# mirage/decompress

Measured on AMD Instinct MI355X. Metric: MiB/s inflate over N zlib streams (uncompressed bytes / wall second), higher is better.
Workload: dtype u8

## Files before the change

decompress_amd/csrc/inflate_wave.hip:

```cpp
#include <stdlib.h>
#include <string.h>
#include "inflate_util.hpp"

namespace md {
namespace wv {

constexpr uint32_t S = 264;
constexpr uint32_t SMIN = 48;
constexpr uint32_t KMAX = 64;
#ifndef MD_EMIT_SPLIT
#define MD_EMIT_SPLIT 1
#endif
#if defined(MD_DEBUG_KNOWN_BOUNDS)
#undef MD_EMIT_SPLIT
#define MD_EMIT_SPLIT 0
#endif
#ifndef MD_SPLIT_B
#define MD_SPLIT_B 4
#endif
#ifndef MD_RUNIN_NUM
#define MD_RUNIN_NUM 3
#define MD_RUNIN_DEN 2
#endif
constexpr uint32_t RUNIN_NUM = MD_RUNIN_NUM, RUNIN_DEN = MD_RUNIN_DEN;
constexpr uint32_t PASSES = 5;
constexpr uint32_t PASS_BITS = 1600, PASSES_MAX = 16;
constexpr uint32_t RMAX = 768;
constexpr uint32_t STAGE = 5568;
constexpr uint32_t WIN_WORDS = 544;

constexpr uint32_t kLitSize = 852, kDistSize = 592;
constexpr uint32_t kLitRootMax = 512;
constexpr uint32_t kLitSubB = 0;
constexpr uint32_t kDistB = kLitSize - kLitRootMax;
constexpr uint32_t kLitB = kDistB + kDistSize;
constexpr uint32_t kStopEobI = kLitB + kLitRootMax;
constexpr uint32_t kStopBadI = kStopEobI + 2;
constexpr uint32_t kLutWords = kStopBadI + 2;
constexpr uint32_t kTbMask = 0xffe00000u;
constexpr uint32_t kLoopy = 0x100u;
static_assert(kDistB % 2 == 0 && kLitB % 2 == 0 && kStopEobI % 2 == 0 && kLutWords == 1448, "even table bases");
constexpr uint32_t kStEob = 100, kStTrunc = 101;
constexpr uint32_t kCountMatch = 1u << 20;
constexpr uint32_t kNearBit = 0x8000u;

struct Mail {
  uint32_t emitted;
  uint32_t copied;
  uint32_t kind;
  uint32_t total;
  uint32_t x;
  uint32_t stuck;
  uint32_t a, b;
};
constexpr uint32_t kJobRound = 0, kJobStored = 1, kJobQuit = 2, kJobEmit = 3;
constexpr uint32_t kHxUni = 4 * 64;
struct Smem {
  uint32_t win[WIN_WORDS];
  uint32_t lut[kLutWords];
  uint32_t mrec[RMAX];
  uint16_t mpos[RMAX];
  alignas(16) uint8_t stage[STAGE + 16];
  uint16_t list[RMAX];
  Mail mail;
};
struct HScratch {
  uint8_t lens[384];
  uint16_t work[320];
  uint32_t ctr;
};
static_assert(sizeof(Smem) <= 20480, "8 streams (16 wavefronts) per CU");
constexpr uint32_t kHScratchAt = 1136;
static_assert(kHScratchAt >= 4 + 572 + 8 && kHScratchAt % 16 == 0 && kHScratchAt + sizeof(HScratch) <= WIN_WORDS * 4, "header scratch lives behind the header's bits");
typedef MD_LDS Smem lds_smem;
typedef MD_LDS HScratch lds_hscratch;
__device__ __forceinline__ lds_hscratch *hscratch_of(lds_smem *sm) {
  return reinterpret_cast<lds_hscratch *>(reinterpret_cast<lds_u8 *>(sm->win) + kHScratchAt);
}

#ifdef MD_DEBUG_KNOWN_BOUNDS
constexpr uint32_t KB_ROUNDS = 512;
__device__ uint4 *g_kb_buf;
__device__ int g_kb_mode;
#endif
__device__ __forceinline__ uint32_t mk_entry(uint32_t n, uint32_t xb, uint32_t val8, uint32_t nbits, uint32_t tb) {
  return n | (xb << 5) | (val8 << 9) | (nbits << 17) | (tb << 21);
}
__device__ __forceinline__ uint32_t e_n(uint32_t e) { return e & 31; }
__device__ __forceinline__ uint32_t e_xb(uint32_t e) { return (e >> 5) & 15; }
__device__ __forceinline__ uint32_t e_val(uint32_t e) { return (e >> 9) & 255; }
__device__ __forceinline__ uint32_t e_tb(uint32_t e) { return e >> 21; }
__device__ __forceinline__ bool e_link(uint32_t e) { return e_tb(e) < kLitB && e_tb(e) != kDistB; }
__device__ __forceinline__ uint32_t e_root(uint32_t lroot) { return mk_entry(0, 0, 0, lroot, kLitB); }
__device__ __forceinline__ uint32_t lit_leaf(uint32_t sym, uint32_t codelen, uint32_t lroot, uint32_t droot) {
  if (sym < 256) return mk_entry(codelen, 0, sym, lroot, kLitB);
  if (sym == 256) return mk_entry(codelen, 0, 0, 0, kStopEobI);
  const uint32_t l = (sym - 257) & 31;
  const uint32_t xb = (l >= 8 && l < 28) ? (l - 4) >> 2 : 0;
  const uint32_t base3 = l < 8 ? l : l < 28 ? (4 + (l & 3)) << xb : l == 28 ? 255 : 0;
  return mk_entry(codelen + xb, xb, base3, droot, kDistB);
}
__device__ __forceinline__ uint32_t dist_leaf(uint32_t dv, uint32_t codelen, uint32_t lroot) {
  dv &= 31;
  if (dv >= 30) return mk_entry(codelen, 0, 0, 0, kStopBadI);
  const uint32_t xb = dv >= 4 ? (dv - 2) >> 1 : 0;
  const uint32_t m = dv < 4 ? dv : ((dv & 1) | 2);
  return mk_entry(codelen + xb, xb, m, lroot, kLitB);
}
__device__ __forceinline__ uint32_t dist_value(uint32_t m, uint32_t xb, uint32_t x) { return (m << xb) + 1 + x; }

struct Window {
  uint32_t w[8], wx;
  uint32_t base;
#ifdef MD_DEBUG_KNOWN_BOUNDS
  uint32_t kb_round, kb_sid;
#endif
  __device__ __forceinline__ void fetch(const uint8_t *__restrict__ body, uint32_t nbytes, uint32_t b, uint32_t lane) {
    base = b;
    const uint32_t off = b + lane * 32;
#pragma unroll
    for (int k = 0; k < 8; k++) w[k] = 0;
    if (off + 32 <= nbytes) __builtin_memcpy(w, body + off, 32);
    else if (off < nbytes)
      for (uint32_t k = 0; k < 32 && off + k < nbytes; k++) w[k >> 2] |= (uint32_t)body[off + k] << (8 * (k & 3));
    wx = 0;
    if (lane < WIN_WORDS - 512) {
      const uint32_t ox = b + 2048 + lane * 4;
      if (ox + 4 <= nbytes) __builtin_memcpy(&wx, body + ox, 4);
      else if (ox < nbytes)
        for (uint32_t k = 0; k < 4 && ox + k < nbytes; k++) wx |= (uint32_t)body[ox + k] << (8 * k);
    }
  }
  __device__ __forceinline__ void put(lds_u32 *win, uint32_t lane) const {
    lds_u32 *dst = win + lane * 8;
#pragma unroll
    for (int k = 0; k < 8; k++) dst[k] = w[k];
    if (lane < WIN_WORDS - 512) win[512 + lane] = wx;
  }
  __device__ __forceinline__ void ensure(lds_u32 *win, const uint8_t *__restrict__ body, uint32_t nbytes, uint32_t b, uint32_t lane) {
    if (base != b) fetch(body, nbytes, b, lane);
    put(win, lane);
    base = 0xffffffffu;
  }
};
__device__ __forceinline__ uint32_t peek(const lds_u32 *win, uint32_t p) {
  const lds_u32 *q = reinterpret_cast<const lds_u32 *>(reinterpret_cast<const lds_u8 *>(win) + ((p >> 3) & ~3u));
  return __builtin_amdgcn_alignbit(q[1], q[0], p & 31);
}
__device__ __forceinline__ uint32_t lut_at(const lds_u32 *lut, uint32_t tb, uint32_t idx) {
  return *reinterpret_cast<const lds_u32 *>(reinterpret_cast<const lds_u8 *>(lut) + ((tb + idx) << 2));
}

struct UBits {
  const lds_u32 *win;
  uint64_t buf;
  uint32_t n;
  uint32_t wp;
  __device__ __forceinline__ void init(const lds_u32 *w, uint32_t bp) {
    win = w;
    wp = bp >> 5;
    buf = ((uint64_t)uni(win[wp]) | ((uint64_t)uni(win[wp + 1]) << 32)) >> (bp & 31);
    n = 64 - (bp & 31);
    wp += 2;
  }
  __device__ __forceinline__ uint32_t pos() const { return wp * 32 - n; }
  __device__ __forceinline__ void fill() {
    if (n <= 32) {
      buf |= (uint64_t)uni(win[wp]) << n;
      n += 32;
      wp++;
    }
  }
  __device__ __forceinline__ uint32_t peekb(uint32_t k) const { return (uint32_t)buf & ((1u << k) - 1); }
  __device__ __forceinline__ void drop(uint32_t k) {
    buf >>= k;
    n -= k;
  }
};

struct Canon {
  uint32_t cnt[16];
  uint32_t first[16];
  uint32_t offs[16];
  uint32_t max, min, root, left;
};
__device__ __forceinline__ uint32_t lane_rank(uint64_t m) {
  return __builtin_amdgcn_mbcnt_hi((uint32_t)(m >> 32), __builtin_amdgcn_mbcnt_lo((uint32_t)m, 0));
}
template <int K>
__device__ __forceinline__ void canon_counts(const uint32_t (&len)[K], uint32_t rootpref, Canon &c) {
#pragma unroll
  for (int l = 1; l < 16; l++) {
    uint32_t n = 0;
#pragma unroll
    for (int k = 0; k < K; k++) n += (uint32_t)__builtin_popcountll(__ballot(len[k] == (uint32_t)l));
    c.cnt[l] = n;
  }
  c.cnt[0] = 0;
  c.max = 0;
  c.min = 16;
#pragma unroll
  for (int l = 15; l >= 1; l--) {
    if (c.cnt[l] && c.max == 0) c.max = l;
    if (c.cnt[l]) c.min = l;
  }
  int left = 1;
  bool over = false;
  uint32_t code = 0, off = 0;
  c.first[0] = 0;
  c.offs[0] = 0;
#pragma unroll
  for (int l = 1; l < 16; l++) {
    left = (left << 1) - (int)c.cnt[l];
    over = over || left < 0;
    code = (code + c.cnt[l - 1]) << 1;
    c.first[l] = code;
    c.offs[l] = off;
    off += c.cnt[l];
  }
  c.left = over ? 0xffffffffu : (uint32_t)left;
  uint32_t root = rootpref;
  if (root > c.max) root = c.max;
  if (root < c.min) root = c.min;
  c.root = root;
// ... 319 lines not shown
  uint32_t e = lut_step(lut, e_root(lroot), w);
  if (e_link(e)) {
    p += e_n(e);
    w = peek(win, p);
    e = lut_step(lut, e, w);
  }
  uint32_t n = e_n(e), xb = e_xb(e), ntb = e_tb(e);
  uint32_t pn = p + n;
  if (pn > tot) return MD_UNEXPECTED_END_OF_INPUT;
  if (ntb == kStopEobI) return kStEob | (pn << 8);
  if (ntb != kDistB) {
    if (q >= cap) return MD_UNEXPECTED_END_OF_OUTPUT;
    return kStTrunc;
  }
  const uint32_t mlen = e_val(e) + 3 + __builtin_amdgcn_ubfe(w, n - xb, xb);
  p = pn;
  w = peek(win, p);
  e = lut_step(lut, e, w);
  if (e_tb(e) == kStopBadI && e_n(e) == 0) return MD_INVALID_DISTANCE_CODE;
  if (e_link(e)) {
    p += e_n(e);
    w = peek(win, p);
    e = lut_step(lut, e, w);
  }
  n = e_n(e), xb = e_xb(e);
  pn = p + n;
  if (pn > tot) return MD_UNEXPECTED_END_OF_INPUT;
  if (e_tb(e) == kStopBadI) return MD_INVALID_DISTANCE_CODE;
  const uint32_t d = dist_value(e_val(e), xb, __builtin_amdgcn_ubfe(w, n - xb, xb));
  const uint32_t lim = q < 32768u ? q : 32768u;
  if (d > lim) return MD_INVALID_DISTANCE;
  if (mlen > cap - q) return MD_UNEXPECTED_END_OF_OUTPUT;
  return kStTrunc;
}

template <bool CHECKED, bool BUDGET>
__device__ __forceinline__ void emit_pass(const lds_u32 *win, const lds_u32 *lut, uint32_t lroot, lds_u32 *mrec,
                                          lds_u16 *mpos, lds_u8 *stage, uint32_t rec0, uint32_t tot, bool go, uint32_t start,
                                          uint32_t limit, uint32_t q0, uint32_t rb, uint32_t R0, uint32_t cap, LaneOut &lo) {
  uint32_t p = start, ptok = start, e = e_root(lroot);
  uint32_t q = q0, rec = rec0, mlen = 0;
  bool stopped = false;
  const uint32_t qlim = rb + STAGE - 16;
  const uint32_t qmax = cap < qlim ? cap : qlim;
  if (go && p < limit) {
    const uint32_t thr = (kLitB << 21) | limit;
    uint32_t slot = 0, key;
    Cursor c;
    c.init(win, start);
    do {
      const uint32_t w = c.peek(p);
      const uint32_t en = lut_step(lut, e, w);
      const uint32_t n = e_n(en), xb = e_xb(en), ntb = e_tb(en);
      const uint32_t x = __builtin_amdgcn_ubfe(w, n - xb, xb);
      const uint32_t pn = p + n;
      const bool to_root = ntb == kLitB, is_len = ntb == kDistB;
      const bool mat = to_root & (mlen != 0), lit = to_root & (mlen == 0);
      const uint32_t d1 = (e_val(en) << xb) + x;
      if (CHECKED) {
        const uint32_t lim = q < 32768u ? q : 32768u;
        const uint32_t need = mat ? mlen : 1u;
        stopped = (ntb >= kStopEobI) | (pn > tot) | (mat & (d1 >= lim)) | (to_root & (q + need > qmax));
        if (stopped) break;
      }
      stage[lit ? q - rb : STAGE + 15] = (uint8_t)(en >> 9);
      if (mat) {
        mrec[rec] = ((mlen - 3) << 16) | ((q - d1 + mlen > R0 + 1) ? kNearBit : 0u) | d1;
        mpos[rec] = (uint16_t)(q - rb);
        rec++;
      }
      q += to_root ? (mlen > 1u ? mlen : 1u) : 0u;
      mlen = is_len ? e_val(en) + 3 + x : to_root ? 0u : mlen;
      p = pn;
      ptok = to_root ? pn : ptok;
      c.seek(win, p);
      e = en;
      key = (en & kTbMask) | p;
      if (BUDGET && ++slot >= KMAX && to_root) break;
    } while (key < thr);
    if (!CHECKED) stopped = e_tb(e) >= kStopEobI;
  }
  uint32_t stopc = 0, endp = p;
  if (go && stopped) {
    const uint32_t r = slow_token(win, lut, lroot, ptok, q, tot, cap);
    stopc = r & 0xffu;
    endp = stopc == kStEob ? r >> 8 : ptok;
  }
  if (go) {
    lo.endp = endp;
    lo.stopc = stopc;
    lo.bytes = q - q0;
    lo.nm = rec - rec0;
  }
}

struct Sink {
  lds_u8 *stage;
  uint8_t *g;
  uint32_t cap;
  uint32_t pos;
  uint32_t lane;
  uint32_t a, b;
  bool want_adler;
  __device__ __forceinline__ uint32_t sbase() const { return pos & ~15u; }

  __device__ __forceinline__ void flush(uint32_t total) {
    const uint32_t rb = sbase();
    const uint32_t endp = pos + total;
    const uint32_t full0 = (pos + 15) & ~15u, full1 = endp & ~15u;
    uint32_t s1 = 0, s2 = 0;
    for (uint32_t ps = full0; ps < full1; ps += 1024) {
      const uint32_t cpos = ps + lane * 16;
      if (cpos < full1) {
        const lds_u32 *sp = reinterpret_cast<const lds_u32 *>(stage + (cpos - rb));
        const uint32_t w0 = sp[0], w1 = sp[1], w2 = sp[2], w3 = sp[3];
        const uint4 v = make_uint4(w0, w1, w2, w3);
        __builtin_memcpy(g + cpos, &v, 16);
        if (want_adler) {
          uint32_t t1 = __builtin_amdgcn_udot4(w0, 0x01010101u, 0u, false);
          t1 = __builtin_amdgcn_udot4(w1, 0x01010101u, t1, false);
          t1 = __builtin_amdgcn_udot4(w2, 0x01010101u, t1, false);
          t1 = __builtin_amdgcn_udot4(w3, 0x01010101u, t1, false);
          uint32_t tk = __builtin_amdgcn_udot4(w0, 0x03020100u, 0u, false);
          tk = __builtin_amdgcn_udot4(w1, 0x07060504u, tk, false);
          tk = __builtin_amdgcn_udot4(w2, 0x0b0a0908u, tk, false);
          tk = __builtin_amdgcn_udot4(w3, 0x0f0e0d0cu, tk, false);
          s1 += t1;
          s2 += (endp - cpos) * t1 - tk;
        }
      }
    }
    {
      const uint32_t head1 = full0 < endp ? full0 : endp;
      const uint32_t tail0 = full1 > head1 ? full1 : head1;
      const uint32_t x = lane < 16 ? pos + lane : tail0 + (lane - 16);
      if (lane < 16 ? x < head1 : (lane < 32 && x < endp)) {
        const uint32_t d = stage[x - rb];
        g[x] = (uint8_t)d;
        s1 += d;
        s2 += (endp - x) * d;
      }
    }
    if (want_adler) {
      s1 = wave_sum(s1);
      s2 = wave_sum(s2 % 65521u);
      b = (b + total * a + s2) % 65521u;
      a = (a + s1) % 65521u;
    }
    pos = endp;
  }
};

constexpr int FR = RMAX / kWave;
struct FarRow {
  uint32_t qs, n, src;
  bool near, has;
  uint32_t ml;
};
__device__ __forceinline__ FarRow far_row(const lds_u32 *mrec, const lds_u16 *mpos, uint32_t r, uint32_t nrec, uint32_t rb, uint32_t R0) {
  FarRow f;
  f.has = r < nrec;
  const uint32_t tk = mrec[f.has ? r : 0u];
  f.qs = mpos[f.has ? r : 0u];
  const uint32_t d = (tk & 0x7fff) + 1;
  f.ml = ((tk >> 16) & 0xff) + 3;
  const uint32_t s = rb + f.qs - d;
  f.near = f.has && (tk & kNearBit);
  const uint32_t head = s < R0 ? R0 - s : 0u;
  f.n = !f.has ? 0u : f.near ? head : f.ml;
  f.src = f.n ? s : 0u;
  return f;
}
template <class PF>
__device__ __forceinline__ void copy_far(const lds_u32 *mrec, const lds_u16 *mpos, lds_u16 *list, const Sink &sk,
                                         uint32_t lane, uint32_t nrec, uint32_t *nnear_out, PF &pf) {
  lds_u8 *stage = sk.stage;
  const uint32_t R0 = sk.pos, rb = sk.sbase();
  const uint8_t *g = sk.g;
  uint32_t nnear = 0;
  uint64_t v0[FR], v1[FR];
  uint32_t pk[FR];
  uint32_t nlong = 0;
  bool spill = false;
#pragma unroll
  for (int u = 0; u < FR; u++) {
    const FarRow f = far_row(mrec, mpos, u * kWave + lane, nrec, rb, R0);
    v0[u] = out_ld64(g + f.src);
    v1[u] = out_ld64(g + f.src + 8);
    pk[u] = f.qs | (f.n << 16);
    const uint64_t nb = __ballot(f.near);
    if (f.near) list[nnear + lane_rank(nb)] = (uint16_t)(u * kWave + lane);
    nnear += (uint32_t)__builtin_popcountll(nb);
    const uint64_t lb = __ballot(f.n > 16);
    const uint32_t lc = (uint32_t)__builtin_popcountll(lb);
    if (nnear + nlong + lc > RMAX) {
      spill = true;
      nlong = 0;
    }
    if (lb && !spill) {
      if (f.n > 16) list[RMAX - 1 - (nlong + lane_rank(lb))] = (uint16_t)(u * kWave + lane);
      nlong += lc;
    }
  }
  pf.tick_lds(P_FAR_REC);
#pragma unroll
  for (int u = 0; u < FR; u++) {
    if ((uint32_t)u * kWave < nrec) {
      const uint32_t qs = pk[u] & 0xffffu, n = pk[u] >> 16;
      if constexpr (PF::on) {
        if (u == 0) {
          asm volatile("" ::"v"(v0[u]), "v"(v1[u]));
          pf.tick_all(P_FAR_LOAD);
        }
      }
      if (n) {
        lds_u8 *dd = stage + qs;
        lds_put(dd, v0[u], n < 8 ? n : 8);
        if (n > 8) lds_put(dd + 8, v1[u], n < 16 ? n - 8 : 8);
      }
    }
  }
  pf.tick_lds(P_FAR);
  for (uint32_t c0 = 0; c0 < nlong; c0 += kWave) {
    const bool has = c0 + lane < nlong;
    const uint32_t r = has ? list[RMAX - 1 - (c0 + lane)] : 0u;
    const FarRow f = far_row(mrec, mpos, r, nrec, rb, R0);
    const uint32_t n = has ? f.n : 0u;
    const uint64_t w0 = out_ld64(g + (n ? f.src + 16 : 0u)), w1 = out_ld64(g + (n ? f.src + 24 : 0u));
    if (n) {
      lds_u8 *dd = stage + f.qs + 16;
      lds_put(dd, w0, n < 24 ? n - 16 : 8);
      if (n > 24) lds_put(dd + 8, w1, n < 32 ? n - 24 : 8);
    }
    for (uint64_t lm = __ballot(n > 32); lm;) {
      uint32_t ln[4], lsrc[4], lqs[4];
      uint64_t d[4];
#pragma unroll
      for (int k = 0; k < 4; k++) {
        const bool any = lm != 0;
        const uint32_t l = any ? (uint32_t)__builtin_ctzll(lm) : 0u;
        lm &= lm - 1;
        ln[k] = any ? rdlane(n, l) : 0u;
        lsrc[k] = rdlane(f.src, l);
        lqs[k] = rdlane(f.qs, l);
      }
      const uint32_t j = 32 + lane * 8;
#pragma unroll
      for (int k = 0; k < 4; k++) d[k] = out_ld64(g + (j < ln[k] ? lsrc[k] + j : 0u));
#pragma unroll
      for (int k = 0; k < 4; k++)
        if (j < ln[k]) lds_put(stage + lqs[k] + j, d[k], ln[k] - j < 8 ? ln[k] - j : 8);
    }
  }
  if (spill) {
    for (uint32_t c0 = 0; c0 < nrec; c0 += kWave) {
      const FarRow f = far_row(mrec, mpos, c0 + lane, nrec, rb, R0);
      for (uint64_t lm = __ballot(f.n > 16); lm; lm &= lm - 1) {
        const uint32_t l = (uint32_t)__builtin_ctzll(lm);
        const uint32_t ln = rdlane(f.n, l), lsrc = rdlane(f.src, l), lqs = rdlane(f.qs, l);
        const uint32_t j = 16 + lane * 8;
        if (j < ln) lds_put(stage + lqs + j, out_ld64(g + lsrc + j), ln - j < 8 ? ln - j : 8);
      }
    }
  }
  pf.tick_all(P_FAR);
  *nnear_out = nnear;
}
template <class PF>
__device__ __noinline__ void copy_far_guarded(const lds_u32 *mrec, const lds_u16 *mpos, lds_u16 *list,
                                              lds_u8 *stage, const uint8_t *g, uint32_t R0, uint32_t rb, uint32_t cap,
                                              uint32_t lane, uint32_t nrec, uint32_t *nnear_out) {
  uint32_t nnear = 0;
  for (uint32_t c0 = 0; c0 < nrec; c0 += kWave) {
    const uint32_t r = c0 + lane;
    const bool has = r < nrec;
    const uint32_t tk = mrec[has ? r : 0u], qs = mpos[has ? r : 0u];
    const uint32_t d = (tk & 0x7fff) + 1, ml = ((tk >> 16) & 0xff) + 3;
    const uint32_t s = rb + qs - d;
    const bool near = has && (tk & kNearBit);
    uint32_t n = has ? ml : 0u;
    const uint64_t nb = __ballot(near);
    if (near) {
      list[nnear + lane_rank(nb)] = (uint16_t)r;
      n = s < R0 ? R0 - s : 0u;
    }
    nnear += (uint32_t)__builtin_popcountll(nb);
    for (uint32_t j = 0; j < n; j += 8) lds_put(stage + qs + j, out_ld_guard(g, s + j, n - j, cap), n - j < 8 ? n - j : 8);
  }
  *nnear_out = nnear;
}

__device__ __forceinline__ void wave_copy(lds_u8 *stage, uint32_t dd, uint32_t ss, uint32_t n, uint32_t d, uint32_t lane) {
  if (d >= n) {
    const uint32_t j = lane * 8;
    if (j < n) lds_put(stage + dd + j, lds_ld64(stage + ss + j), n - j < 8 ? n - j : 8);
  } else if (d < 8) {
    uint64_t v = lds_ld64(stage + ss);
    const uint32_t sh = 8 * d;
    v &= (1ull << sh) - 1;
    v |= v << sh;
    if (2 * sh < 64) v |= v << (2 * sh);
    if (4 * sh < 64) v |= v << (4 * sh);
    const uint32_t adv = (0x76586880u >> (4 * d)) & 15;
    const uint32_t j = lane * adv;
    if (j < n) lds_put(stage + dd + j, v, n - j < adv ? n - j : adv);
  } else {
    const float inv = 1.0f / (float)d;
    for (uint32_t j = lane * 4; j < n; j += 4 * kWave) {
      uint32_t r = j - (uint32_t)((float)j * inv) * d;
      r = (int32_t)r < 0 ? r + d : r;
      r = r >= d ? r - d : r;
      uint32_t w = 0;
#pragma unroll
      for (uint32_t k = 0; k < 4; k++) {
        const uint32_t x = r + k >= d ? r + k - d : r + k;
        w |= (uint32_t)stage[ss + x] << (8 * k);
      }
      lds_put(stage + dd + j, w, n - j < 4 ? n - j : 4);
    }
  }
}

template <class PF>
__device__ __forceinline__ void copy_near_all(const lds_u32 *mrec, const lds_u16 *mpos, const lds_u16 *list,
                                              const Sink &sk, uint32_t lane, uint32_t count, bool *stuck, PF &pf) {
  lds_u8 *stage = sk.stage;
  const uint32_t head = sk.pos - sk.sbase();
  for (uint32_t c0 = 0; c0 < count; c0 += kWave) {
    bool todo = c0 + lane < count;
    const uint32_t e = todo ? list[c0 + lane] : 0u;
    const uint32_t tk = mrec[e], qs = mpos[e];
    const uint32_t d = (tk & 0x7fff) + 1, ml = ((tk >> 16) & 0xff) + 3;
    const int32_t s0 = (int32_t)qs - (int32_t)d;
    const uint32_t skip = s0 < (int32_t)head ? head - (uint32_t)s0 : 0u;
    const uint32_t sa = (uint32_t)(s0 + (int32_t)skip), sb = d < ml ? qs : (uint32_t)s0 + ml;
    const uint32_t n = ml - skip;
    const bool fast = d >= n && n <= 32;
    const uint32_t qb = todo ? qs + skip : 0xffffffffu, qe = todo ? qs + ml : 0xffffffffu;
    uint32_t jlo = 0, jhi = 0;
#pragma unroll
    for (uint32_t st = 32; st > 0; st >>= 1) {
      const uint32_t ve = __shfl(qe, jlo + st - 1), vb = __shfl(qb, jhi + st - 1);
      jlo = ve <= sa ? jlo + st : jlo;
      jhi = vb < sb ? jhi + st : jhi;
    }
    jhi = jhi < lane ? jhi : lane;
    uint64_t need = 0;
    if (sa < sb && jlo < jhi) need = ((jhi >= 64 ? 0ull : (1ull << jhi)) - 1ull) & ~((1ull << jlo) - 1ull);
    uint64_t done = 0;
    pf.tick_lds(P_NEAR_LOAD);
    for (uint32_t guard = 0; __ballot(todo) != 0; guard++) {
      if (guard > kWave) {
        *stuck = true;
        return;
      }
      pf.count(C_NEAR_IT);
      const bool ready = todo && (need & ~done) == 0;
      if constexpr (PF::on) {
        if (__ballot(ready && !fast)) pf.count(C_LONG_NEAR);
      }
      pf.tick_lds(P_NEAR);
      if (ready && fast) {
        lds_u8 *dd = stage + qs + skip;
        const lds_u8 *ss = stage + sa;
        const uint64_t v0 = lds_ld64(ss), v1 = lds_ld64(ss + 8), v2 = lds_ld64(ss + 16), v3 = lds_ld64(ss + 24);
        lds_put(dd, v0, n < 8 ? n : 8);
        if (n > 8) lds_put(dd + 8, v1, n < 16 ? n - 8 : 8);
        if (n > 16) {
          lds_put(dd + 16, v2, n < 24 ? n - 16 : 8);
          if (n > 24) lds_put(dd + 24, v3, n - 24);
        }
      }
// ... 156 lines not shown
    }
    bool split = false;
    uint32_t bq = 0, br = 0;
    LaneOut lob;
    lob.endp = 0, lob.stopc = 0, lob.bytes = 0, lob.nm = 0;
    bool gob = false;
    if constexpr (kSplit) split = zs >= 128;
    {
      const uint32_t all = rdlane(off + mynb, nvalid - 1) & (kCountMatch - 1);
      const bool plain = tot >= rbp + kWave * zs + 64 && R0 >= 32768u && all <= sk.cap - R0 && (R0 - rb) + all <= STAGE - 16;
      uint32_t alimit = limit;
      if constexpr (kSplit) {
        if (split) {
          gob = mine && midp != 0xffffffffu && midp < limit && midp >= start;
          bq = midcnt & (kCountMatch - 1);
          br = midcnt >> 20;
          lds_u32 *hx = reinterpret_cast<lds_u32 *>(sm->list);
          hx[4 * lane + 0] = gob ? midp : 0xffffffffu;
          hx[4 * lane + 1] = limit;
          hx[4 * lane + 2] = q0 + bq;
          hx[4 * lane + 3] = roff + br;
          if (lane < 6) hx[kHxUni + lane] = lane == 0 ? lroot : lane == 1 ? tot : lane == 2 ? rb : lane == 3 ? R0 : lane == 4 ? sk.cap : (plain ? 0u : 1u);
          mail_post(sm, lane, kJobEmit, 0, 0, sent);
          alimit = gob ? midp : limit;
        }
      }
      if (plain && !BUDGET) emit_pass<false, false>(win, lut, lroot, mrec, mpos, sk.stage, roff, tot, mine, start, alimit, q0, rb, R0, sk.cap, lo);
      else emit_pass<true, BUDGET>(win, lut, lroot, mrec, mpos, sk.stage, roff, tot, mine, start, alimit, q0, rb, R0, sk.cap, lo);
      if constexpr (kSplit) {
        if (split) {
          if (!mail_wait_idle(sm, sent)) return MD_E_HIP;
          const lds_u32 *hx = reinterpret_cast<const lds_u32 *>(sm->list);
          if (gob) {
            lob.endp = hx[4 * lane + 0];
            lob.stopc = hx[4 * lane + 1];
            lob.bytes = hx[4 * lane + 2];
            lob.nm = hx[4 * lane + 3];
          }
          const bool sa = lo.stopc != 0;
          if (!sa && gob) {
            lo.endp = lob.endp;
            lo.stopc = lob.stopc;
            lo.bytes = bq + lob.bytes;
            lo.nm = br + lob.nm;
          }
        }
      }
    }
    pf.tick(P_EMIT_A);
    uint32_t total, lstop, nrec;
    {
      const uint64_t fm = __ballot(mine && lo.stopc != 0);
      if (fm) {
        const uint32_t fl = __builtin_ctzll(fm);
        lstop = rdlane(lo.stopc, fl);
        total = rdlane(boff, fl) + rdlane(lo.bytes, fl);
        nrec = rdlane(roff, fl) + rdlane(lo.nm, fl);
        if (lstop == kStEob) pf.count(C_END_EOB);
        else if (lstop == kStTrunc) pf.count(C_END_STAGE);
        nvalid = fl + 1;
      } else {
        lstop = 0;
        const uint32_t all = rdlane(off + mynb, nvalid - 1);
        total = all & (kCountMatch - 1);
        nrec = all >> 20;
      }
    }
    const uint32_t nbp = base * 8 + rdlane(lo.endp, nvalid - 1);
    wnd.fetch(body, body_len, (nbp >> 5) << 2, lane);
    bool stuck = false;
    if constexpr (PAIR) {
      mail_post(sm, lane, kJobRound, total, nrec, sent);
      sk.pos += total;
    } else {
      copy_round(sm, sk, lane, total, nrec, &stuck, pf);
    }
    pf.count(C_LANES, nvalid);
    if (stuck || (nbp == bp && total == 0 && (lstop == 0 || lstop == kStTrunc))) return MD_E_HIP;
    {
      const uint32_t bits = nbp - bp;
      const uint64_t want = (uint64_t)(STAGE - STAGE / 8) * bits / ((uint64_t)kWave * (total ? total : 1u));
      zs = want > S ? S : want < SMIN ? SMIN : (uint32_t)want;
    }
    bp = nbp;
    if (lstop == kStEob) break;
    if (lstop != 0 && lstop != kStTrunc) return (int)lstop;
  }
  *bp_io = bp;
  *zone_io = zs;
  return MD_OK;
}

__device__ __forceinline__ void copy_stored(Sink &sk, const uint8_t *__restrict__ body, uint32_t p, uint32_t len, uint32_t lane) {
  const uint8_t *q = body + p;
  uint32_t left = len;
  while (left) {
    const uint32_t seg = left < STAGE - 16 ? left : STAGE - 16;
    const uint32_t s0 = sk.pos - sk.sbase();
    for (uint32_t j = lane; j < seg; j += kWave) sk.stage[s0 + j] = q[j];
    sk.flush(seg);
    q += seg;
    left -= seg;
  }
}

template <class PF>
__device__ __forceinline__ void copier_main(lds_smem *sm, const uint8_t *__restrict__ body, Sink &sk, uint32_t lane, PF &pf) {
  uint32_t done = 0;
  for (;;) {
    while (uni(mail_ld(&sm->mail.emitted)) == done) __builtin_amdgcn_s_sleep(2);
    asm volatile("" ::: "memory");
    const uint32_t kind = uni(sm->mail.kind), total = uni(sm->mail.total), x = uni(sm->mail.x);
    pf.tick(P_WAIT_COPY);
    if (kind == kJobQuit) break;
    bool stuck = false;
    if (kind == kJobRound) copy_round(sm, sk, lane, total, x, &stuck, pf);
    else if (kind == kJobEmit) {
      if constexpr (MD_EMIT_SPLIT != 0) {
        lds_u32 *hx = reinterpret_cast<lds_u32 *>(sm->list);
        const uint32_t bstart = hx[4 * lane + 0], blimit = hx[4 * lane + 1], bq0 = hx[4 * lane + 2], brec = hx[4 * lane + 3];
        const uint32_t lroot = uni(hx[kHxUni + 0]), tot = uni(hx[kHxUni + 1]), rb = uni(hx[kHxUni + 2]), R0 = uni(hx[kHxUni + 3]),
                       cap = uni(hx[kHxUni + 4]), checked = uni(hx[kHxUni + 5]);
        const bool go = bstart != 0xffffffffu;
        LaneOut lo;
        lo.endp = bstart, lo.stopc = 0, lo.bytes = 0, lo.nm = 0;
        const lds_u32 *win = (const lds_u32 *)sm->win;
        const lds_u32 *lut = (const lds_u32 *)sm->lut;
        if (checked) emit_pass<true, false>(win, lut, lroot, (lds_u32 *)sm->mrec, (lds_u16 *)sm->mpos, sk.stage, brec, tot, go, go ? bstart : 0u, blimit, bq0, rb, R0, cap, lo);
        else emit_pass<false, false>(win, lut, lroot, (lds_u32 *)sm->mrec, (lds_u16 *)sm->mpos, sk.stage, brec, tot, go, go ? bstart : 0u, blimit, bq0, rb, R0, cap, lo);
        hx[4 * lane + 0] = lo.endp;
        hx[4 * lane + 1] = lo.stopc;
        hx[4 * lane + 2] = lo.bytes;
        hx[4 * lane + 3] = lo.nm;
      }
    } else copy_stored(sk, body, x, total, lane);
    if (lane == 0) {
      sm->mail.a = sk.a;
      sm->mail.b = sk.b;
      if (stuck) sm->mail.stuck = 1;
    }
    asm volatile("s_waitcnt lgkmcnt(0)" ::: "memory");
    done++;
    if (lane == 0) mail_st(&sm->mail.copied, done);
  }
}

struct Cont {
  const uint32_t *start_bit, *hist_len, *adler_in;
  uint64_t *resume_bits, *resume_out;
  uint32_t *resume_adler, *resume_last;
};

template <bool PROF, bool PAIR>
__global__ __launch_bounds__(PAIR ? 2 * kWave : kWave, PAIR ? 4 : 2) void inflate_wave_kernel(
    int format, uint32_t n, const uint8_t *__restrict__ in, const uint64_t *__restrict__ in_off,
    const uint64_t *__restrict__ in_len, uint8_t *out, const uint64_t *__restrict__ out_off,
    const uint64_t *__restrict__ out_cap, uint64_t *__restrict__ out_len,
    uint64_t *__restrict__ consumed, int32_t *__restrict__ status, uint32_t *__restrict__ checksum,
    uint64_t *__restrict__ dbg, const uint32_t *__restrict__ order, Cont cont) {
  __shared__ Smem smem;
  lds_smem *sm = (lds_smem *)&smem;
  Prof<PROF> pf;
  pf.init();
  const uint32_t lane = threadIdx.x & (kWave - 1);
  const uint32_t wave = PAIR ? uni(threadIdx.x / kWave) : 0u;
  if (blockIdx.x >= n) return;
  const uint32_t sid = order ? order[blockIdx.x] : blockIdx.x;

  const uint8_t *src = in + in_off[sid];
  uint64_t slen64 = in_len[sid], cap64 = out_cap[sid];
  if (slen64 > MD_MAX_INFLATE_IN) {
    if (threadIdx.x == 0) {
      out_len[sid] = 0;
      consumed[sid] = 0;
      status[sid] = MD_E_INVALID_ARGUMENT;
      if (checksum) checksum[sid] = 0;
    }
    return;
  }
  const uint32_t slen = (uint32_t)slen64;
  const bool cap_clamped = cap64 > MD_MAX_STREAM;
  const uint32_t cap = cap_clamped ? (uint32_t)MD_MAX_STREAM : (uint32_t)cap64;

  int rc = MD_OK;
  uint32_t body_off = 0, body_len = slen;
  if (format == MD_FORMAT_ZLIB) {
    if (slen < 2) rc = MD_UNEXPECTED_END_OF_INPUT;
    else {
      uint32_t cmf = src[0], flg = src[1];
      if (((cmf << 8) + flg) % 31 != 0 || (cmf & 0xf) != 8) rc = MD_INVALID_HEADER;
      else if (slen < 6) rc = MD_UNEXPECTED_END_OF_INPUT;
      else {
        body_off = 2;
        body_len = slen - 6;
      }
    }
  }
  const uint8_t *body = src + body_off;

  Sink sk;
  sk.stage = (lds_u8 *)sm->stage;
  sk.g = out + out_off[sid];
  sk.cap = cap;
  const uint32_t hist = cont.hist_len ? cont.hist_len[sid] : 0u, adler0 = cont.adler_in ? cont.adler_in[sid] : 1u;
  sk.pos = hist < cap ? hist : cap;
  sk.lane = lane;
  sk.a = adler0 & 0xffffu;
  sk.b = adler0 >> 16;
  sk.want_adler = (checksum != nullptr) || format == MD_FORMAT_ZLIB || cont.resume_adler != nullptr;

  if (threadIdx.x < 4) sm->lut[kStopEobI + threadIdx.x] = mk_entry(0, 0, 0, 0, kStopEobI + (threadIdx.x & 2));
  if constexpr (PAIR) {
    if (threadIdx.x < sizeof(Mail) / 4) ((lds_u32 *)&sm->mail)[threadIdx.x] = threadIdx.x == 6 ? sk.a : threadIdx.x == 7 ? sk.b : 0u;
    __syncthreads();
    if (wave == 1) {
      copier_main(sm, body, sk, lane, pf);
      if constexpr (PROF) {
        if (lane == 0 && sid == 0 && dbg) {
          const int mine[] = {P_FAR, P_NEAR, P_ADLER, P_NEAR_FAST, P_NEAR_SLOW, P_NEAR_UPD, P_NEAR_LOAD, P_FAR_REC, P_FAR_LOAD, P_WAIT_COPY};
          for (int i : mine) dbg[i] = pf.acc[i];
          dbg[P_COUNT + C_NEAR_IT] = pf.cnt[C_NEAR_IT];
          dbg[P_COUNT + C_LONG_NEAR] = pf.cnt[C_LONG_NEAR];
        }
      }
      return;
    }
  }

  lds_u32 *win = (lds_u32 *)sm->win;
  const uint32_t total_bits = body_len * 8;
  uint32_t bp = cont.start_bit ? cont.start_bit[sid] & 7u : 0u;
  uint32_t zone = S;
  uint32_t sent = 0;
  uint32_t fixed_lroot = 0;
  Window wnd;
  wnd.base = 0xffffffffu;
#ifdef MD_DEBUG_KNOWN_BOUNDS
  wnd.kb_round = 0;
  wnd.kb_sid = sid;
#endif
  if (cont.resume_bits && lane == 0) {
    cont.resume_bits[sid] = bp;
    cont.resume_out[sid] = sk.pos;
    cont.resume_adler[sid] = adler0;
    cont.resume_last[sid] = 0;
  }

  if (rc == MD_OK) {
    bool last = false;
    uint32_t lds_base = 0xffffffffu;
    while (!last && rc == MD_OK) {
      uint32_t base = (bp >> 5) << 2;
      if (lds_base != 0xffffffffu && bp >= lds_base * 8 && bp - lds_base * 8 <= 4096) base = lds_base;
      else {
        wnd.ensure(win, body, body_len, base, lane);
        lds_base = base;
      }
      uint32_t rbp = bp - base * 8;
      const uint32_t tot = total_bits - base * 8;
      if ((int32_t)(tot - rbp) < 3) {
        rc = MD_UNEXPECTED_END_OF_INPUT;
        break;
      }
      const uint32_t hdr = uni(peek(win, rbp));
      last = hdr & 1;
      uint32_t type = (hdr >> 1) & 3;
      bp += 3;
      rbp += 3;
      bool block_done = false;
      if (type == 1) {
        for (;;) {
          if (rbp + 7 > tot || rbp + 64 > WIN_WORDS * 32 - 64 || (uni(peek(win, rbp)) & 0x7fu) != 0) break;
          rbp += 7;
          bp += 7;
          block_done = true;
          if (last || rbp + 3 > tot) break;
          const uint32_t h = uni(peek(win, rbp)) & 7u;
          if (((h >> 1) & 3) != 1) break;
          last = h & 1;
          rbp += 3;
          bp += 3;
          block_done = false;
        }
      }
      if (block_done) {
      } else if (type == 0) {
        uint32_t p = (bp + 7) >> 3;
        if (body_len - p < 4) {
          rc = MD_UNEXPECTED_END_OF_INPUT;
          break;
        }
        uint32_t h4;
        if (p + 4 <= base + (WIN_WORDS - 2) * 4) h4 = uni(peek(win, (p - base) * 8));
        else h4 = (uint32_t)body[p] | ((uint32_t)body[p + 1] << 8) | ((uint32_t)body[p + 2] << 16) | ((uint32_t)body[p + 3] << 24);
        uint32_t len = h4 & 0xffff, nlen = h4 >> 16;
        p += 4;
        if (nlen != 0xffff - len) rc = MD_INVALID_COMPLEMENT_OF_LENGTH;
        else if (len > body_len - p) rc = MD_UNEXPECTED_END_OF_INPUT;
        else if (len > sk.cap - sk.pos) rc = MD_UNEXPECTED_END_OF_OUTPUT;
        else {
          if (len) {
            if constexpr (PAIR) {
              if (!mail_wait_idle(sm, sent)) rc = MD_E_HIP;
              mail_post(sm, lane, kJobStored, len, p, sent);
              sk.pos += len;
            } else {
              copy_stored(sk, body, p, len, lane);
// ... 182 lines not shown
```

Before: 243,100.

## Shrink record and stage buffers to fit nine streams per CU; ring-buffer far loads

Reduces RMAX from 768 to 576 and STAGE from 5568 to 5296 so the per-stream LDS footprint allows nine streams (18 wavefronts) per CU, and raises the launch-bounds occupancy hint to match. The far-copy loop is software-pipelined with an 8-deep ring of register buffers instead of holding all FR rows' loads, which lowers VGPR pressure to support the higher occupancy. Smaller record and staging buffers mean fewer matches per round, so there may be more rounds and extra per-round overhead.

After: 248,100, median of 6. 1.02x the previous value.

```diff
diff --git a/decompress_amd/csrc/inflate_wave.hip b/decompress_amd/csrc/inflate_wave.hip
--- a/decompress_amd/csrc/inflate_wave.hip
+++ b/decompress_amd/csrc/inflate_wave.hip
@@ -25,8 +25,14 @@
 constexpr uint32_t RUNIN_NUM = MD_RUNIN_NUM, RUNIN_DEN = MD_RUNIN_DEN;
 constexpr uint32_t PASSES = 5;
 constexpr uint32_t PASS_BITS = 1600, PASSES_MAX = 16;
-constexpr uint32_t RMAX = 768;
-constexpr uint32_t STAGE = 5568;
+#ifndef MD_RMAX
+#define MD_RMAX 576
+#endif
+#ifndef MD_STAGE
+#define MD_STAGE 5296
+#endif
+constexpr uint32_t RMAX = MD_RMAX;
+constexpr uint32_t STAGE = MD_STAGE;
 constexpr uint32_t WIN_WORDS = 544;
 
 constexpr uint32_t kLitSize = 852, kDistSize = 592;
@@ -69,7 +75,14 @@
   uint16_t work[320];
   uint32_t ctr;
 };
-static_assert(sizeof(Smem) <= 20480, "8 streams (16 wavefronts) per CU");
+static_assert(sizeof(Smem) <= 20480, "at least 8 streams (16 wavefronts) per CU");
+static_assert(RMAX % 64 == 0 && STAGE % 16 == 0 && RMAX * 2 >= (kHxUni + 6) * 4, "record rows, staging chunks, hand-over");
+constexpr uint32_t kSmemAlloc = (sizeof(Smem) + 511) / 512 * 512;
+constexpr uint32_t kStreamsPerCU = 160 * 1024 / kSmemAlloc;
+constexpr uint32_t kPairWavesPerSimd = (kStreamsPerCU + 1) / 2;
+#if MD_RMAX == 576 && MD_STAGE == 5296
+static_assert(kStreamsPerCU == 9, "the shipped layout: 9 streams (18 wavefronts) per CU");
+#endif
 constexpr uint32_t kHScratchAt = 1136;
 static_assert(kHScratchAt >= 4 + 572 + 8 && kHScratchAt % 16 == 0 && kHScratchAt + sizeof(HScratch) <= WIN_WORDS * 4, "header scratch lives behind the header's bits");
 typedef MD_LDS Smem lds_smem;
@@ -695,6 +708,7 @@
 };
 
 constexpr int FR = RMAX / kWave;
+constexpr int FB = 8;
 struct FarRow {
   uint32_t qs, n, src;
   bool near, has;
@@ -721,46 +735,49 @@
   const uint32_t R0 = sk.pos, rb = sk.sbase();
   const uint8_t *g = sk.g;
   uint32_t nnear = 0;
-  uint64_t v0[FR], v1[FR];
-  uint32_t pk[FR];
+  uint64_t v0[FB], v1[FB];
+  uint32_t pk[FB];
   uint32_t nlong = 0;
   bool spill = false;
 #pragma unroll
-  for (int u = 0; u < FR; u++) {
-    const FarRow f = far_row(mrec, mpos, u * kWave + lane, nrec, rb, R0);
-    v0[u] = out_ld64(g + f.src);
-    v1[u] = out_ld64(g + f.src + 8);
-    pk[u] = f.qs | (f.n << 16);
-    const uint64_t nb = __ballot(f.near);
-    if (f.near) list[nnear + lane_rank(nb)] = (uint16_t)(u * kWave + lane);
-    nnear += (uint32_t)__builtin_popcountll(nb);
-    const uint64_t lb = __ballot(f.n > 16);
-    const uint32_t lc = (uint32_t)__builtin_popcountll(lb);
-    if (nnear + nlong + lc > RMAX) {
-      spill = true;
-      nlong = 0;
-    }
-    if (lb && !spill) {
-      if (f.n > 16) list[RMAX - 1 - (nlong + lane_rank(lb))] = (uint16_t)(u * kWave + lane);
-      nlong += lc;
-    }
-  }
-  pf.tick_lds(P_FAR_REC);
-#pragma unroll
-  for (int u = 0; u < FR; u++) {
-    if ((uint32_t)u * kWave < nrec) {
-      const uint32_t qs = pk[u] & 0xffffu, n = pk[u] >> 16;
-      if constexpr (PF::on) {
-        if (u == 0) {
-          asm volatile("" ::"v"(v0[u]), "v"(v1[u]));
-          pf.tick_all(P_FAR_LOAD);
-        }
-      }
-      if (n) {
-        lds_u8 *dd = stage + qs;
-        lds_put(dd, v0[u], n < 8 ? n : 8);
-        if (n > 8) lds_put(dd + 8, v1[u], n < 16 ? n - 8 : 8);
-      }
+  for (int t = 0; t < FR + FB; t++) {
+    if (t >= FB) {
+      const int u = t - FB;
+      if ((uint32_t)u * kWave < nrec) {
+        const uint32_t qs = pk[u % FB] & 0xffffu, n = pk[u % FB] >> 16;
+        if constexpr (PF::on) {
+          if (u == 0) {
+            asm volatile("" ::"v"(v0[0]), "v"(v1[0]));
+            pf.tick_all(P_FAR_LOAD);
+          }
+        }
+        if (n) {
+          lds_u8 *dd = stage + qs;
+          lds_put(dd, v0[u % FB], n < 8 ? n : 8);
+          if (n > 8) lds_put(dd + 8, v1[u % FB], n < 16 ? n - 8 : 8);
+        }
+      }
+    }
+    if (t < FR) {
+      const int u = t;
+      const FarRow f = far_row(mrec, mpos, u * kWave + lane, nrec, rb, R0);
+      v0[u % FB] = out_ld64(g + f.src);
+      v1[u % FB] = out_ld64(g + f.src + 8);
+      pk[u % FB] = f.qs | (f.n << 16);
+      const uint64_t nb = __ballot(f.near);
+      if (f.near) list[nnear + lane_rank(nb)] = (uint16_t)(u * kWave + lane);
+      nnear += (uint32_t)__builtin_popcountll(nb);
+      const uint64_t lb = __ballot(f.n > 16);
+      const uint32_t lc = (uint32_t)__builtin_popcountll(lb);
+      if (nnear + nlong + lc > RMAX) {
+        spill = true;
+        nlong = 0;
+      }
+      if (lb && !spill) {
+        if (f.n > 16) list[RMAX - 1 - (nlong + lane_rank(lb))] = (uint16_t)(u * kWave + lane);
+        nlong += lc;
+      }
+      if (u == (FB < FR ? FB : FR) - 1) pf.tick_lds(P_FAR_REC);
     }
   }
   pf.tick_lds(P_FAR);
@@ -1223,7 +1240,7 @@
 };
 
 template <bool PROF, bool PAIR>
-__global__ __launch_bounds__(PAIR ? 2 * kWave : kWave, PAIR ? 4 : 2) void inflate_wave_kernel(
+__global__ __launch_bounds__(PAIR ? 2 * kWave : kWave, PAIR ? kPairWavesPerSimd : 2) void inflate_wave_kernel(
     int format, uint32_t n, const uint8_t *__restrict__ in, const uint64_t *__restrict__ in_off,
     const uint64_t *__restrict__ in_len, uint8_t *out, const uint64_t *__restrict__ out_off,
     const uint64_t *__restrict__ out_cap, uint64_t *__restrict__ out_len,
```
